# X-rayLaser/DistributedLLM

Hardware: NVIDIA H100
Metric: decode tokens/sec LLaMA-7B Q4_0 seq512 bs1 (higher is better)
Workload: dtype q4_0*q8_0->f32

## Files before the change

### distributedllm_b200/capi.py

```python
from __future__ import annotations

import ctypes as C
import os
from typing import Optional

import numpy as np

HERE = os.path.dirname(os.path.abspath(__file__))
LIB_PATH = os.path.join(HERE, "libb200slice.so")

ERRORS = {1: "EINVAL", 2: "EFILE", 3: "ENODEV", 4: "ECUDA", 5: "ECONTEXT", 6: "ENCCL"}


class B200Error(RuntimeError):
    def __init__(self, code: int, msg: str):
        super().__init__("b200 error %d (%s): %s" % (code, ERRORS.get(code, "?"), msg))
        self.code = code


class SliceInfo(C.Structure):
    _fields_ = [(n, C.c_int32) for n in ("n_embd", "n_head", "n_ff", "n_layer", "first_layer", "n_ctx", "n_past",
                                          "weight_type", "device")] + [("weight_bytes", C.c_int64),
                                                                        ("kv_bytes_per_pos", C.c_int64)]

# ... 36 lines not shown
        L.b200_slice_sync.argtypes = [vp]
        L.b200_slice_last_ms.argtypes = [vp]
        L.b200_slice_last_ms.restype = cf
        L.b200_slice_launch_count.argtypes = [vp]
        L.b200_slice_launch_count.restype = C.c_int64
        L.b200_slice_set_fast_prefill.argtypes = [vp, ci, ci]
        L.b200_slice_mark.argtypes = [vp, ci]
        L.b200_slice_mark_elapsed_ms.argtypes = [vp]
        L.b200_slice_mark_elapsed_ms.restype = cf
        L.b200_slice_profile.argtypes = [vp, ci]
        L.b200_slice_profile_read.argtypes = [vp, vp, vp, ci]
        L.b200_debug_read.argtypes = [vp, ci, C.c_size_t, C.c_size_t, vp]
        L.b200_debug_trace_enable.argtypes = [vp, ci]
        L.b200_debug_skip_attention.argtypes = [vp, ci]
        L.b200_debug_trace_read.argtypes = [vp, vp, vp, vp, ci]
        L.b200_slice_dev_in.argtypes = [vp]
        L.b200_slice_dev_in.restype = vp
        L.b200_slice_dev_out.argtypes = [vp]
        L.b200_slice_dev_out.restype = vp
        L.b200_pipeline_result.argtypes = [vp]
        L.b200_pipeline_result.restype = vp
        L.b200_device_init.argtypes = [ci]
        for name, args in (("b200_pipeline_unique_id", [vp]), ("b200_pipeline_init", [vp, ci, ci, vp]),
                           ("b200_pipeline_step", [vp, vp, ci, ci]),
                           ("b200_pipeline_mailbox_export", [vp, vp]), ("b200_pipeline_mailbox_connect", [vp, vp, ci]),
                           ("b200_pipeline_collect", [vp, ci, vp]), ("b200_pipeline_pingpong", [vp, ci, ci, vp]), ("b200_pipeline_transport", [vp]), ("b200_pipeline_set_transport", [vp, ci]), ("b200_pipeline_error", [vp]),
                           ("b200_pipeline_step_session", [vp, ci, vp, ci, ci]), ("b200_pipeline_step_batch", [vp, vp, ci, vp, ci]),
                           ("b200_pipeline_step_mixed", [vp, vp, vp, ci, vp, ci]), ("b200_pipeline_destroy", [vp]),
                           ("b200_extra_load", [C.c_char_p, ci, C.POINTER(vp)]), ("b200_extra_unload", [vp]),
                           ("b200_extra_dims", [vp, C.POINTER(ci), C.POINTER(ci)]),
# ... 153 lines not shown
        return out.view(dtype)

    def skip_attention(self, on: bool) -> None:
        check(lib().b200_debug_skip_attention(self._h, int(on)))

    def trace_enable(self, on: bool) -> None:
        check(lib().b200_debug_trace_enable(self._h, int(on)))

    def trace_read(self, max_launches: int = 512):
        buf = np.zeros((max_launches, 1024, 8), np.uint64)
        cls = np.zeros(max_launches, np.int32)
        ctas = np.zeros(max_launches, np.int32)
        n = lib().b200_debug_trace_read(self._h, _ptr(buf), _ptr(cls), _ptr(ctas), max_launches)
        return buf[:n], cls[:n], ctas[:n]

    def last_ms(self) -> float:
        return float(lib().b200_slice_last_ms(self._h))

    def launch_count(self) -> int:
        return int(lib().b200_slice_launch_count(self._h))

    def close(self) -> None:
        if self._h:
            check(lib().b200_slice_unload(self._h))
            self._h = C.c_void_p()

    def __del__(self):
        try:
            self.close()
        except Exception:
# ... 139 lines not shown
```

### distributedllm_b200/csrc/kernels.cuh

```cuda
#pragma once
#include "common.cuh"

namespace b200 {

constexpr int kWT_F16 = 1, kWT_Q4_0 = 2, kWT_Q4_1 = 3, kWT_Q5_0 = 6, kWT_Q5_1 = 7, kWT_Q8_0 = 8;
constexpr int kQ4Chunk = 576, kQ41Chunk = 640, kQ50Chunk = 704, kQ51Chunk = 768, kQ8Chunk = 1088;
constexpr int kWPC = 4;
constexpr int kConsumers = kWPC * 32;
constexpr int kQS = 4;
constexpr float kMagic = 12582912.0f;
constexpr int kMagicI = 0x4B400000;

struct WtTraits {
    int block_bytes;
    int chunk_bytes;
    bool is_signed;
    bool min_plane;
    bool high_plane;
    bool q8_1;
    float act_scale;
};
__host__ __device__ constexpr WtTraits wt_traits(int wt) {
    return wt == kWT_Q4_0 ? WtTraits{18, kQ4Chunk, true, false, false, false, 0.0625f}
         : wt == kWT_Q4_1 ? WtTraits{20, kQ41Chunk, false, true, false, true, 0.0625f}
// ... 267 lines not shown
    const int tid = threadIdx.x, warp = tid >> 5, lane = tid & 31;
    const int col0 = blockIdx.y * NC;
    const int n_stage = nbq / kQS;

    if (tid == 0) {
        B200_TRACE(a.trace, 0);
        if (RING) for (int s = 0; s < NS; s++) { mbar_init(&full[s], 1); mbar_init(&empty[s], kWPC); }
        mbar_init(actbar, 1);
        mbar_init(actbar + 1, kWPC);
        mbar_fence_init();
    }
    __syncthreads();

    if (RING && warp == kWPC) {
        if (lane == 0) {
            int slot = 0, use = 0, issued = 0;
            for (int tile = blockIdx.x; tile < a.W.n_tiles; tile += gridDim.x) {
                const uint8_t * src = a.W.data + (long long) tile * a.W.tile_bytes;
                for (int s = 0; s < n_stage; s++) {
                    if (issued == a.pre_stages) mbar_wait(actbar + 1, 0);
                    issued++;
                    if (use > 0) mbar_wait(&empty[slot], (use - 1) & 1);
                    mbar_arrive_expect_tx(&full[slot], (uint32_t) stage_bytes);
                    bulk_g2s(ring + (size_t) slot * stage_bytes, src + (size_t) s * stage_bytes, (uint32_t) stage_bytes, &full[slot]);
                    if (++slot == NS) { slot = 0; use++; }
                }
            }
            if (issued <= a.pre_stages) mbar_wait(actbar + 1, 0);
            grid_dep_launch();
            B200_TRACE(a.trace, 4);
        }
        return;
    }

    float wn[32];
    if (PRO == PRO_NORM && nb <= kConsumers) {
        #pragma unroll
        for (int j = 0; j < 8; j++) {
            const float4 u = tid < nb ? ldg_keep(a.norm_w + tid * 32 + (((NC == 1 ? tid : 0) + j) & 7) * 4) : make_float4(0.f, 0.f, 0.f, 0.f);
            wn[j*4] = u.x; wn[j*4+1] = u.y; wn[j*4+2] = u.z; wn[j*4+3] = u.w;
        }
    }
    grid_dep_wait();
    if (!RING && tid == 0) grid_dep_launch();
// ... 1323 lines not shown
```

### distributedllm_b200/csrc/kquant.cuh

```cuda
#pragma once
#include "kernels.cuh"

namespace b200 {

constexpr int kWT_Q4_K = 12;
constexpr int kQ4KChunk = 1152, kQ6KChunk = 1680;
constexpr int kKQS = 2;
static_assert(kQ4KChunk == 8 * 144 && kQ6KChunk == 8 * 210, "a chunk holds the file's bytes, nothing added");
static_assert(kQ4KChunk % 16 == 0 && kQ6KChunk % 16 == 0, "a ring stage stays one bulk copy");

__host__ __device__ constexpr bool wt_kquant(int wt) { return wt == kWT_Q4_K || wt == kWT_Q6_K; }
__host__ __device__ constexpr int kq_chunk_bytes(int wt) { return wt == kWT_Q4_K ? kQ4KChunk : kQ6KChunk; }
__host__ __device__ constexpr int kq_block_bytes(int wt) { return wt == kWT_Q4_K ? 144 : 210; }

__global__ void k_repack_kq(RepackArgs a) {
    const int cb = kq_chunk_bytes(a.wtype), words = cb / 4, bsz = kq_block_bytes(a.wtype);
    const bool q6 = a.wtype == kWT_Q6_K;
    const long long total = (long long) a.n_tiles * a.nbq * a.TR * words;
    for (long long i = blockIdx.x * (long long) blockDim.x + threadIdx.x; i < total; i += (long long) gridDim.x * blockDim.x) {
        const int wi = (int)(i % words);
        long long c = i / words;
        const int rg = (int)(c % a.TR); c /= a.TR;
        const int sb = (int)(c % a.nbq);
        const int tile = (int)(c / a.nbq);
// ... 130 lines not shown
    const int tid = threadIdx.x, warp = tid >> 5, lane = tid & 31;
    const int col0 = blockIdx.y * NC;
    const int n_stage = nbq / kKQS;

    if (tid == 0) {
        B200_TRACE(a.trace, 0);
        if (RING) for (int s = 0; s < NS; s++) { mbar_init(&full[s], 1); mbar_init(&empty[s], kWPC); }
        mbar_init(actbar, 1);
        mbar_init(actbar + 1, kWPC);
        mbar_fence_init();
    }
    __syncthreads();

    if (RING && warp == kWPC) {
        if (lane == 0) {
            int slot = 0, use = 0, issued = 0;
            for (int tile = blockIdx.x; tile < a.W.n_tiles; tile += gridDim.x) {
                const uint8_t * src = a.W.data + (long long) tile * a.W.tile_bytes;
                for (int s = 0; s < n_stage; s++) {
                    if (issued == a.pre_stages) mbar_wait(actbar + 1, 0);
                    issued++;
                    if (use > 0) mbar_wait(&empty[slot], (use - 1) & 1);
                    mbar_arrive_expect_tx(&full[slot], (uint32_t) stage_bytes);
                    bulk_g2s(ring + (size_t) slot * stage_bytes, src + (size_t) s * stage_bytes, (uint32_t) stage_bytes, &full[slot]);
                    if (++slot == NS) { slot = 0; use++; }
                }
            }
            if (issued <= a.pre_stages) mbar_wait(actbar + 1, 0);
            grid_dep_launch();
            B200_TRACE(a.trace, 4);
        }
        return;
    }

    grid_dep_wait();
    if (!RING && tid == 0) grid_dep_launch();
    if (tid == 0) B200_TRACE(a.trace, 1);

    const int ncols = min(NC, a.N - col0);
    if (tid == 0) {
        const uint32_t b1 = (uint32_t) ncols * nbq * 256, b2 = (uint32_t) ncols * nbq * 32, b3 = (uint32_t) ncols * nbd * 4;
        mbar_arrive_expect_tx(actbar, b1 + b2 + b3);
        bulk_g2s(aq_s, a.aq_in + (size_t) col0 * nbq * 64, b1, actbar);
        bulk_g2s(as_s, a.aq_in + a.in_soff + (size_t) col0 * nbq * 8, b2, actbar);
// ... 175 lines not shown
```

### distributedllm_b200/csrc/runtime.cu

```cuda
#include "kernels.cuh"
#include "kquant.cuh"
#include "fastgemm2.cuh"
#include "ggjt_file.hpp"

#include <algorithm>
#include <atomic>
#include <chrono>
#include <climits>
#include <cmath>
#include <condition_variable>
#include <dlfcn.h>
#include <cstdlib>
#include <map>
#include <memory>
#include <mutex>
#include <thread>
#include <type_traits>
#include <vector>

namespace b200 {

constexpr int kSmemLimit = 226 * 1024;

struct LayerW {
    PackedW qkv{}, wo{}, w13{}, w2{};
    PackedW qkv_more[2]{}; int qkv_row[2] = {0, 0};
    uint16_t * f_q = nullptr, * f_k = nullptr, * f_v = nullptr, * f_o = nullptr, * f_1 = nullptr, * f_2 = nullptr, * f_3 = nullptr;
    float * attn_norm = nullptr, * ffn_norm = nullptr;
};

struct GraphKey { const float * in; float * out; int host; bool operator<(const GraphKey & o) const {
    return in != o.in ? in < o.in : (out != o.out ? out < o.out : host < o.host); } };

}

using namespace b200;

struct b200_slice {
    int device = 0, n_sm = 132;
    cudaStream_t stream = nullptr;
    int E = 0, H = 0, D = 0, FF = 0, L = 0, first_layer = 0, n_ctx = 512, wtype = 0;
// ... 10 lines not shown
    uint16_t * kc = nullptr, * vc = nullptr, * q16 = nullptr;
    float * xa = nullptr, * xb = nullptr, * qkv = nullptr, * att = nullptr, * ffin = nullptr, * gate = nullptr;
    float * d_in = nullptr, * d_out = nullptr, * h_in = nullptr, * h_out = nullptr;
    float2 * cs = nullptr; uint16_t * texp = nullptr, * tsilu = nullptr;
    int * aq_att = nullptr, * aq_gate = nullptr; float * da_att = nullptr, * da_gate = nullptr;
    int nbqE = 0, nbqF = 0;
    int soffE = 0, soffF = 0;
    int * aq_x = nullptr; float * da_x = nullptr; int * nq_counter = nullptr; double * nq_partial = nullptr;
    std::map<GraphKey, cudaGraphExec_t> graphs;
    cudaEvent_t ev0 = nullptr, ev1 = nullptr; bool timed = false;
    int64_t launches = 0, weight_bytes = 0;
    bool use_ring = true, use_graph = true, use_pdl = false, use_nq = true, f16_ring = true, use_tiled_attn = true, f16_mc = true; int f16_mc_cols = 4;
    bool skip_attention = false;
    bool attn_lut_smem = true;
    bool fast_prefill = false; int fast_min_tokens = 32; uint16_t * xh = nullptr;
    int opt_ns = 0, opt_cta_per_sm = 0, opt_nc = 0, opt_pre = 3, opt_nomath = 0;
    float ema_token_ms = 0.f;
    std::mutex mu;
    bool profiling = false; int cur_class = 0;
    std::vector<cudaEvent_t> prof_ev; std::vector<int> prof_cls; size_t prof_used = 0;
    cudaEvent_t mark[2] = {nullptr, nullptr};
    unsigned long long * trace = nullptr; int trace_next = 0; std::vector<int> trace_cls, trace_ctas;
    void * nccl_comm = nullptr; int pp_rank = 0, pp_world = 1; float * d_final = nullptr;
    uint8_t * mb_block = nullptr; size_t mb_slot_floats = 0;
    uint8_t * mb_next = nullptr, * mb_prev = nullptr; bool mb_on = false;
    bool send_pending = false; PeerSendArgs send_args{}; int send_ctas = 1;
    bool fold_send = false, use_fold = true;
    int * kq_aq = nullptr; float * kq_ad = nullptr;
    std::map<GraphKey, cudaGraphExec_t> pp_graphs;
};

// ... 80 lines not shown
        m.act = kq_act_bytes(W.nbq, NC) + 34 * 8 + 64;
        return m;
    }
    m.stage = (size_t) kQS * kWPC * G * chunk_bytes(WT);
    m.act = (size_t) NC * act_bytes_per_col(W.nbq, WT) + 34 * 8 + kWPC * 8 + (size_t) NC * 128 + 64 +
            ((NC == 1 && PRO == PRO_NORM) ? (size_t) W.K * 4 : 0);
    return m;
}

template <int WT, int G, int NC, int PRO, int EPI, bool RING>
static constexpr auto gemv_kernel() {
    if constexpr (wt_kquant(WT)) return k_gemv_kq<WT, G, NC, PRO, EPI, RING>;
    else return k_gemv<WT, G, NC, PRO, EPI, RING>;
}

template <int WT, int G, int NC, int PRO, int EPI, bool RING>
static int launch_gemv_t(b200_slice * s, GemvArgs a) {
    constexpr auto kern = gemv_kernel<WT, G, NC, PRO, EPI, RING>();
    const GemvSmem sm = gemv_smem<WT, G, NC, PRO>(a.W);
    const size_t stage = sm.stage, act = sm.act;
    int NS = 0;
    if (RING) {
        const int ncolg = (a.N + NC - 1) / NC;
        int need = (a.W.n_tiles * ncolg + s->n_sm - 1) / s->n_sm;
        if (need > 5) need = 5;
        const size_t budget = (size_t) kSmemLimit / need - 1024;
        NS = s->opt_ns > 0 ? s->opt_ns : (budget > act ? (int)((budget - act) / stage) : 2);
        if (NS < 2) NS = 2;
        if (NS > 16) NS = 16;
        while (NS > 2 && NS * stage + act > (size_t) kSmemLimit) NS--;
    }
    const size_t smem = sm.bytes(NS);
    if (smem > (size_t) kSmemLimit) return fail(B200_EINVAL, "gemv needs %zu B of shared memory (K=%d, NC=%d)", smem, a.W.K, NC);
    if (int rc = smem_attr<kern>(s, kSmemLimit, true)) return rc;
    a.NS = NS; a.dbg_nomath = s->opt_nomath; a.pre_stages = s->opt_pre;
    a.trace = nullptr;
    if (s->trace && s->trace_next < 512) { a.trace = s->trace + (size_t) s->trace_next * 1024 * 8; s->trace_next++; s->trace_cls.push_back(s->cur_class); }
    int per_sm = s->opt_cta_per_sm > 0 ? s->opt_cta_per_sm : (int)(kSmemLimit / (smem + 1024));
    if (per_sm < 1) per_sm = 1;
    if (per_sm > 6) per_sm = 6;
    const int ncol = (a.N + NC - 1) / NC;
    int gx = a.W.n_tiles;
    const int cap = s->n_sm * per_sm;
    if (gx > cap) gx = cap;
    if (a.trace) s->trace_ctas.push_back(gx * ncol);
    return launch(s, kern, dim3(gx, ncol, 1), dim3(RING ? kConsumers + 32 : kConsumers, 1, 1), smem, a);
}

template <int WT, int G, int PRO, int EPI>
static int launch_gemv_nc(b200_slice * s, const GemvArgs & a) {
    if (a.N == 1) return s->use_ring ? launch_gemv_t<WT, G, 1, PRO, EPI, true>(s, a) : launch_gemv_t<WT, G, 1, PRO, EPI, false>(s, a);
    if (!s->use_ring) return launch_gemv_t<WT, G, 8, PRO, EPI, false>(s, a);
    const int want = 3 * s->n_sm, nt = a.W.n_tiles;
    const int force = s->opt_nc, cap = force > 0 ? force : 8;
    if (cap >= 8 && gemv_smem<WT, G, 8, PRO>(a.W).bytes(2) <= (size_t) kSmemLimit && (force || nt * ((a.N + 7) / 8) >= want))
        return launch_gemv_t<WT, G, 8, PRO, EPI, true>(s, a);
    if (cap >= 4 && gemv_smem<WT, G, 4, PRO>(a.W).bytes(2) <= (size_t) kSmemLimit && (force || nt * ((a.N + 3) / 4) >= want))
        return launch_gemv_t<WT, G, 4, PRO, EPI, true>(s, a);
    return launch_gemv_t<WT, G, 2, PRO, EPI, true>(s, a);
// ... 249 lines not shown
    if ((rc = attention(s, il, N, false))) return rc;
    s->cur_class = 3;
    GemvF16Args o{}; o.K = E; o.x = s->att; o.ldx = E; o.N = N; o.tsilu = s->tsilu;
    o.rows = E; o.W = Lw.f_o; o.resid = cur; o.ldr = E; o.y = s->ffin; o.ldy = E;
    if ((rc = launch_f16<PRO_PLAIN, EPI_RESID>(s, o))) return rc;
    s->cur_class = 4;
    GemvF16Args g{}; g.K = E; g.x = s->ffin; g.ldx = E; g.norm_w = Lw.ffn_norm; g.N = N; g.tsilu = s->tsilu;
    g.rows = FF; g.W = Lw.f_1; g.W2 = Lw.f_3; g.y = s->gate; g.ldy = FF;
    if ((rc = launch_f16<PRO_NORM, EPI_GATE>(s, g))) return rc;
    s->cur_class = 5;
    GemvF16Args w{}; w.K = FF; w.x = s->gate; w.ldx = FF; w.N = N; w.tsilu = s->tsilu;
    w.rows = E; w.W = Lw.f_2; w.resid = s->ffin; w.ldr = E; w.y = nxt; w.ldy = E;
    return launch_f16<PRO_PLAIN, EPI_RESID>(s, w);
}

static int layer_exact(b200_slice * s, int il, int N, const float * cur, float * nxt) {
    const int E = s->E, FF = s->FF;
    const LayerW & Lw = s->layers[il];
    const bool nq = s->use_nq && N == 1 && !s->cols && Lw.wo.n_tiles <= 256 && Lw.wo.n_tiles <= s->n_sm * 2;
    const float dsc = wt_act_scale(s->wtype);
    int rc;
    GemvArgs q{}; q.W = Lw.qkv; q.x = cur; q.ldx = E; q.norm_w = Lw.attn_norm; q.y = s->qkv; q.ldy = 3 * E;
    q.N = N; q.out_rows = 3 * E; q.tsilu = s->tsilu; q.aq_in = s->aq_x; q.da_in = s->da_x; q.in_soff = s->soffE;
    if (N > 1 && (rc = launch_norm_quant(s, cur, E, Lw.attn_norm, N))) return rc;
    if ((rc = N > 1 || (il > 0 && nq) ? launch_gemv<1, PRO_PREQ, EPI_STORE>(s, q) : launch_gemv<1, PRO_NORM, EPI_STORE>(s, q))) return rc;
    if ((rc = attention(s, il, N, true))) return rc;
    s->cur_class = 3;
    GemvArgs o{}; o.W = Lw.wo; o.x = s->att; o.ldx = E; o.resid = cur; o.ldr = E; o.y = s->ffin; o.ldy = E;
    o.N = N; o.out_rows = E; o.tsilu = s->tsilu; o.aq_in = s->aq_att; o.da_in = s->da_att; o.in_soff = s->soffE; o.out_soff = s->soffE;
    o.nq_norm_w = Lw.ffn_norm; o.nq_counter = s->nq_counter; o.nq_partial = s->nq_partial; o.aq_out = s->aq_x; o.da_out = s->da_x; o.out_nbq = s->nbqE; o.out_dscale = dsc;
    if (s->D == 128) rc = nq ? launch_gemv<1, PRO_PREQ, EPI_RESID_NQ>(s, o) : launch_gemv<1, PRO_PREQ, EPI_RESID>(s, o);
    else             rc = nq ? launch_gemv<1, PRO_PLAIN, EPI_RESID_NQ>(s, o) : launch_gemv<1, PRO_PLAIN, EPI_RESID>(s, o);
    if (rc) return rc;
    s->cur_class = 4;
    GemvArgs g{}; g.W = Lw.w13; g.x = s->ffin; g.ldx = E; g.norm_w = Lw.ffn_norm; g.y = s->gate; g.ldy = FF;
    g.N = N; g.out_rows = FF; g.tsilu = s->tsilu; g.aq_in = s->aq_x; g.da_in = s->da_x; g.in_soff = s->soffE; g.out_soff = s->soffF;
    g.aq_out = s->aq_gate; g.da_out = s->da_gate; g.out_nbq = s->nbqF; g.out_dscale = dsc;
    if (N > 1 && (rc = launch_norm_quant(s, s->ffin, E, Lw.ffn_norm, N))) return rc;
    if ((rc = N > 1 || nq ? launch_gemv<2, PRO_PREQ, EPI_GATEQ>(s, g) : launch_gemv<2, PRO_NORM, EPI_GATEQ>(s, g))) return rc;
    s->cur_class = 5;
    GemvArgs w{}; w.W = Lw.w2; w.resid = s->ffin; w.ldr = E; w.y = nxt; w.ldy = E;
    w.N = N; w.out_rows = E; w.tsilu = s->tsilu; w.aq_in = s->aq_gate; w.da_in = s->da_gate; w.in_soff = s->soffF; w.out_soff = s->soffE;
    if (il + 1 < s->L && nq) {
        w.nq_norm_w = s->layers[il + 1].attn_norm; w.nq_counter = s->nq_counter; w.nq_partial = s->nq_partial; w.aq_out = s->aq_x; w.da_out = s->da_x;
        w.out_nbq = s->nbqE; w.out_dscale = dsc;
        return launch_gemv<1, PRO_PREQ, EPI_RESID_NQ>(s, w);
    }
    if (s->fold_send && il == s->L - 1) return launch_w2_send<false>(s, w);
    return launch_gemv<1, PRO_PREQ, EPI_RESID>(s, w);
}

static int layer_fast(b200_slice * s, int il, int N, const float * cur, float * nxt) {
    const int E = s->E, FF = s->FF;
    const LayerW & Lw = s->layers[il];
    int rc;
    if ((rc = launch_prep<true>(s, cur, E, Lw.attn_norm, E, N))) return rc;
    if ((rc = launch_fast_gemm<FG_STORE>(s, Lw.qkv, nullptr, 0, s->qkv, 3 * E, N, 3 * E))) return rc;
    if ((rc = attention(s, il, N, true))) return rc;
    s->cur_class = 3;
    if ((rc = launch_prep<false>(s, s->att, E, nullptr, E, N))) return rc;
    if ((rc = launch_fast_gemm<FG_RESID>(s, Lw.wo, cur, E, s->ffin, E, N, E))) return rc;
    s->cur_class = 4;
    if ((rc = launch_prep<true>(s, s->ffin, E, Lw.ffn_norm, E, N))) return rc;
    if ((rc = launch_fast_gemm<FG_GATE>(s, Lw.w13, nullptr, 0, s->gate, FF, N, FF))) return rc;
    s->cur_class = 5;
    if ((rc = launch_prep<false>(s, s->gate, FF, nullptr, FF, N))) return rc;
    return launch_fast_gemm<FG_RESID>(s, Lw.w2, s->ffin, E, nxt, E, N, E);
}

static int layer_kquant(b200_slice * s, int il, int N, const float * cur, float * nxt) {
    const int E = s->E, FF = s->FF;
    const LayerW & Lw = s->layers[il];
    int rc;
    GemvArgs q{}; q.W = Lw.qkv; q.x = cur; q.ldx = E; q.norm_w = Lw.attn_norm; q.y = s->qkv; q.ldy = 3 * E;
    q.N = N; q.out_rows = Lw.qkv.rows; q.tsilu = s->tsilu;
    if ((rc = quant_kq(s, q, true)) || (rc = launch_gemv_kq<1, PRO_PREQ, EPI_STORE>(s, q))) return rc;
    for (int i = 0; i < 2 && Lw.qkv_more[i].data; i++) {
        q.W = Lw.qkv_more[i]; q.y = s->qkv + Lw.qkv_row[i]; q.out_rows = Lw.qkv_more[i].rows;
        if ((rc = launch_gemv_kq<1, PRO_PREQ, EPI_STORE>(s, q))) return rc;
    }
    if ((rc = attention(s, il, N, false))) return rc;
    s->cur_class = 3;
    GemvArgs o{}; o.W = Lw.wo; o.x = s->att; o.ldx = E; o.resid = cur; o.ldr = E; o.y = s->ffin; o.ldy = E;
    o.N = N; o.out_rows = E; o.tsilu = s->tsilu;
    if ((rc = quant_kq(s, o, false)) || (rc = launch_gemv_kq<1, PRO_PREQ, EPI_RESID>(s, o))) return rc;
    s->cur_class = 4;
    GemvArgs g{}; g.W = Lw.w13; g.x = s->ffin; g.ldx = E; g.norm_w = Lw.ffn_norm; g.y = s->gate; g.ldy = FF;
    g.N = N; g.out_rows = FF; g.tsilu = s->tsilu;
    if ((rc = quant_kq(s, g, true)) || (rc = launch_gemv_kq<2, PRO_PREQ, EPI_GATE>(s, g))) return rc;
    s->cur_class = 5;
    GemvArgs w{}; w.W = Lw.w2; w.x = s->gate; w.ldx = FF; w.resid = s->ffin; w.ldr = E; w.y = nxt; w.ldy = E;
    w.N = N; w.out_rows = E; w.tsilu = s->tsilu;
    if ((rc = quant_kq(s, w, false))) return rc;
    if (s->fold_send && il == s->L - 1) return launch_w2_send<true>(s, w);
    return launch_gemv_kq<1, PRO_PREQ, EPI_RESID>(s, w);
}

static int enqueue_layers(b200_slice * s, const float * in, int N, float * out) {
    const float * cur = in;
    int rc;
    for (int il = 0; il < s->L; il++) {
        const LayerW & Lw = s->layers[il];
        float * nxt = (il == s->L - 1) ? out : ((il & 1) ? s->xb : s->xa);
        const bool fast = s->fast_prefill && N > 1 && !s->cols && N >= s->fast_min_tokens &&
                          (s->wtype == kWT_Q4_0 || s->wtype == kWT_Q8_0) &&
                          (Lw.qkv.n_tiles * Lw.qkv.TR) % 16 == 0 &&
                          (Lw.wo.n_tiles * Lw.wo.TR) % 16 == 0 && (Lw.w13.n_tiles * Lw.w13.TR) % 16 == 0;
// ... 8 lines not shown
    s->cur_class = 6;
    if (s->send_pending) {
        s->send_pending = false;
        if ((rc = launch(s, k_peer_send, dim3(s->send_ctas, 1, 1), dim3(1024, 1, 1), 0, s->send_args))) return rc;
    }
    if (s->cols) return launch(s, k_advance_segs, dim3(1), dim3(32), 0, s->d_npast, s->d_segs, (int) s->segs.size());
    if (s->fold_send) return launch(s, k_advance_sent, dim3(1), dim3(32), 0, s->d_npast + s->cur, N, (MailboxHdr *) s->mb_block);
    return launch(s, k_advance, dim3(1), dim3(32), 0, s->d_npast + s->cur, N);
}

static int step_launches(const b200_slice * s) {
    int n = (s->D == 128 ? 5 : 6) * s->L + 1;
    for (const LayerW & Lw : s->layers) n += (Lw.qkv_more[0].data ? 1 : 0) + (Lw.qkv_more[1].data ? 1 : 0);
    if (wt_kquant(s->wtype)) n += 4 * s->L;
    return n;
}

static int run_decode_graph(b200_slice * s, const float * in, float * out, bool host) {
    GraphKey key{in, out, (host ? 1 : 0) | (s->skip_attention ? 2 : 0) | (s->send_pending ? 4 : 0) | (s->cur << 3)};
    auto it = s->graphs.find(key);
    const int per_step = step_launches(s);
    if (it == s->graphs.end()) {
        const int64_t before = s->launches;
        cudaGraph_t g = nullptr;
        B200_CUDA(cudaStreamBeginCapture(s->stream, cudaStreamCaptureModeThreadLocal));
        int rc = 0;
        if (host) {
            cudaMemcpyAsync(s->d_in, s->h_in, (size_t) s->E * 4, cudaMemcpyHostToDevice, s->stream);
            rc = enqueue_layers(s, s->d_in, 1, s->d_out);
            cudaMemcpyAsync(s->h_out, s->d_out, (size_t) s->E * 4, cudaMemcpyDeviceToHost, s->stream);
// ... 437 lines not shown
        if ((rc = dev_alloc(s, &s->trace, (size_t) 512 * 1024 * 8))) return rc;
        B200_CUDA(cudaMemset(s->trace, 0, (size_t) 512 * 1024 * 8 * 8));
    }
    B200_CUDA(cudaFuncSetAttribute(k_attention, cudaFuncAttributeMaxDynamicSharedMemorySize, kSmemLimit));
    B200_CUDA(cudaFuncSetAttribute(k_attn128<true>, cudaFuncAttributeMaxDynamicSharedMemorySize, 200 * 1024));
    B200_CUDA(cudaFuncSetAttribute(k_attn128<false>, cudaFuncAttributeMaxDynamicSharedMemorySize, 200 * 1024));
    if (s->D == 128) {
        cudaLaunchConfig_t cfg{};
        cfg.gridDim = dim3(4 * s->H, 1, 1); cfg.blockDim = dim3(256, 1, 1); cfg.dynamicSmemBytes = attn_need;
        int clusters = 0;
        B200_CUDA(cudaOccupancyMaxActiveClusters(&clusters, k_attn128<true>, &cfg));
        s->attn_lut_smem = clusters >= s->H;
        if (ltrace) fprintf(stderr, "[b200 load] single-token attention: %d of %d clusters resident with the exp table in shared memory: %s\n",
                            clusters, s->H, s->attn_lut_smem ? "staged" : "read through L2");
    }
    B200_CUDA(cudaEventCreate(&s->ev0));
    B200_CUDA(cudaEventCreate(&s->ev1));
    B200_CUDA(cudaDeviceSynchronize());
    lap("attributes + final sync");
    if (ltrace) fprintf(stderr, "[b200 load] total %.3f s for %.2f GB of weights\n", tnow() - t_begin, s->weight_bytes / 1e9);
    return 0;
}

static void destroy(b200_slice * s) {
    cudaSetDevice(s->device);
    if (s->stream) cudaStreamSynchronize(s->stream);
    for (auto & kv : s->graphs) cudaGraphExecDestroy(kv.second);
    for (auto & kv : s->pp_graphs) cudaGraphExecDestroy(kv.second);
    if (s->mb_next) cudaIpcCloseMemHandle(s->mb_next);
    if (s->mb_prev && s->mb_prev != s->mb_next) cudaIpcCloseMemHandle(s->mb_prev);
// ... 29 lines not shown
    if (device < 0 || device >= ndev) return fail(B200_ENODEV, "device %d out of range (%d visible)", device, ndev);
    cudaDeviceProp prop;
    B200_CUDA(cudaGetDeviceProperties(&prop, device));
    if (prop.major != 9 || prop.minor != 0) return fail(B200_ENODEV, "device %d is sm_%d%d; this library is built for sm_90a only", device, prop.major, prop.minor);
    B200_CUDA(cudaSetDevice(device));
    b200_slice * s = new b200_slice();
    s->device = device; s->n_sm = prop.multiProcessorCount;
    s->n_ctx = n_ctx > 0 ? n_ctx : 512;
    s->n_sessions = n_sessions;
    s->use_ring  = env_int("B200_RING", 1) != 0;
    s->use_graph = env_int("B200_GRAPH", 1) != 0;
    s->use_pdl   = env_int("B200_PDL", 1) != 0;
    s->fast_prefill = env_int("B200_FAST_PREFILL", 0) != 0; s->fast_min_tokens = env_int("B200_FAST_MIN_TOKENS", 32);
    s->use_nq    = env_int("B200_NQ", 0) != 0;
    s->opt_ns = env_int("B200_NS", 0); s->opt_cta_per_sm = env_int("B200_CTA_PER_SM", 0); s->opt_nc = env_int("B200_NC", 0);
    s->opt_pre = env_int("B200_PRE", 3); s->opt_nomath = env_int("B200_DBG_NOMATH", 0);
    s->use_tiled_attn = env_int("B200_TILED_ATTN", 1) != 0;
    s->f16_mc = env_int("B200_F16_MC", 1) != 0;
    s->f16_mc_cols = env_int("B200_F16_MC", 1) == 8 ? 8 : 4;
    s->f16_ring = env_int("B200_F16_RING", 1) != 0;
    cudaError_t e = cudaStreamCreateWithFlags(&s->stream, cudaStreamNonBlocking);
    if (e != cudaSuccess) { delete s; return fail(B200_ECUDA, "cudaStreamCreate failed: %s", cudaGetErrorString(e)); }
    int rc = load_locked(s, path);
    if (rc) { destroy(s); return rc; }
    *out = s;
    return 0;
}

int b200_slice_unload(b200_slice_t * s) {
    if (!s) return fail(B200_EINVAL, "null handle");
    { std::lock_guard<std::mutex> lk(s->mu); }
// ... 225 lines not shown
            else { int rc = dev_alloc(s, &s->trace, (size_t) 512 * 1024 * 8); if (rc) return rc; }
        }
        B200_CUDA(cudaMemset(s->trace, 0, (size_t) 512 * 1024 * 8 * 8));
        s->trace_next = 0; s->trace_cls.clear(); s->trace_ctas.clear();
    } else if (s->trace) { parked = s->trace; s->trace = nullptr; }
    return 0;
}

int b200_debug_trace_read(b200_slice_t * s, unsigned long long * out, int * cls, int * ctas, int max_launches) {
    if (!s || !s->trace) return 0;
    cudaSetDevice(s->device);
    cudaStreamSynchronize(s->stream);
    int n = s->trace_next < max_launches ? s->trace_next : max_launches;
    cudaMemcpy(out, s->trace, (size_t) n * 1024 * 8 * 8, cudaMemcpyDeviceToHost);
    for (int i = 0; i < n; i++) { cls[i] = s->trace_cls[i]; ctas[i] = s->trace_ctas[i]; }
    return n;
}

int b200_debug_read(b200_slice_t * s, int which, size_t offset_words, size_t count, void * out) {
    if (!s || !out) return fail(B200_EINVAL, "null argument");
    const void * src[10] = {s->qkv, s->att, s->ffin, s->gate, s->xa, s->xb, s->q16, s->kc, s->vc, s->xh};
    if (which < 0 || which > 9) return fail(B200_EINVAL, "bad buffer id %d", which);
    B200_CUDA(cudaSetDevice(s->device));
    B200_CUDA(cudaStreamSynchronize(s->stream));
    B200_CUDA(cudaMemcpy(out, (const uint32_t *) src[which] + offset_words, count * 4, cudaMemcpyDeviceToHost));
    return 0;
}

}

// ... 1227 lines not shown
```

### include/b200_slice.h

```cpp
#ifndef B200_SLICE_H
#define B200_SLICE_H

#include <stddef.h>
#include <stdint.h>

#ifdef __cplusplus
extern "C" {
#endif

typedef struct b200_slice b200_slice_t;
typedef struct b200_extra b200_extra_t;

enum {
    B200_OK       = 0,
    B200_EINVAL   = 1,
    B200_EFILE    = 2,
    B200_ENODEV   = 3,
    B200_ECUDA    = 4,
    B200_ECONTEXT = 5,
    B200_ENCCL    = 6,
};

typedef struct b200_slice_info {
    int32_t n_embd, n_head, n_ff, n_layer, first_layer, n_ctx, n_past, weight_type, device;
// ... 46 lines not shown
int b200_slice_profile(b200_slice_t * s, int enable);
int b200_slice_profile_read(b200_slice_t * s, float * ms_by_class, int * launches_by_class, int n_class);

int64_t b200_slice_launch_count(b200_slice_t * s);

float * b200_slice_dev_in(b200_slice_t * s);
float * b200_slice_dev_out(b200_slice_t * s);

int b200_debug_read(b200_slice_t * s, int which, size_t offset_words, size_t count, void * out);

int b200_debug_skip_attention(b200_slice_t * s, int on);

int b200_debug_trace_enable(b200_slice_t * s, int on);
int b200_debug_trace_read(b200_slice_t * s, unsigned long long * out, int * cls, int * ctas, int max_launches);


int b200_pipeline_unique_id(void * id128);
int b200_pipeline_init(b200_slice_t * s, int rank, int nranks, const void * id128);

int b200_pipeline_step(b200_slice_t * s, const float * d_in, int n_tokens, int ring);
int b200_pipeline_step_session(b200_slice_t * s, int session, const float * d_in, int n_tokens, int ring);
int b200_pipeline_step_batch(b200_slice_t * s, const int * sessions, int n_seq, const float * d_in, int ring);
int b200_pipeline_step_mixed(b200_slice_t * s, const int * sessions, const int * counts, int n_seq, const float * d_in, int ring);
int b200_pipeline_mailbox_export(b200_slice_t * s, void * handle64);
int b200_pipeline_mailbox_connect(b200_slice_t * s, const void * handles , int nranks);
int b200_pipeline_transport(b200_slice_t * s);
int b200_pipeline_set_transport(b200_slice_t * s, int peer);
int b200_pipeline_pingpong(b200_slice_t * s, int n_rows, int iters, float * us_per_iter);
int b200_pipeline_error(b200_slice_t * s);

// ... 41 lines not shown
```

Before: 559.3.

## Plan per-launch ring depths and release dependent grid after activation gate

Adds an optional load-time planner that picks a ring depth per decode GEMV, shrinking adjacent launches' shared-memory footprints so consecutive kernels (and attention) can co-reside on an SM under programmatic dependent launch. The producer warp now triggers grid_dep_launch right after the activation gate instead of after issuing all weight loads, letting the next kernel start earlier. The default prefetch depth before the gate changes from 3 to 5 stages (or NS when planned). The planner is off by default (env flag), but the earlier launch trigger and the new prefetch default are always on, which risks the next kernel competing for SMs and bandwidth.

```diff
diff --git a/distributedllm_b200/capi.py b/distributedllm_b200/capi.py
--- a/distributedllm_b200/capi.py
+++ b/distributedllm_b200/capi.py
@@ -74,6 +74,7 @@
         L.b200_debug_trace_enable.argtypes = [vp, ci]
         L.b200_debug_skip_attention.argtypes = [vp, ci]
         L.b200_debug_trace_read.argtypes = [vp, vp, vp, vp, ci]
+        L.b200_debug_ring_plan.argtypes = [vp, vp, ci]
         L.b200_slice_dev_in.argtypes = [vp]
         L.b200_slice_dev_in.restype = vp
         L.b200_slice_dev_out.argtypes = [vp]
@@ -257,6 +258,13 @@
         n = lib().b200_debug_trace_read(self._h, _ptr(buf), _ptr(cls), _ptr(ctas), max_launches)
         return buf[:n], cls[:n], ctas[:n]
 
+    def ring_plan(self) -> np.ndarray:
+        n = lib().b200_debug_ring_plan(self._h, None, 0)
+        check(min(n, 0))
+        out = np.zeros((n, 3), np.int32)
+        lib().b200_debug_ring_plan(self._h, _ptr(out), n)
+        return out
+
     def last_ms(self) -> float:
         return float(lib().b200_slice_last_ms(self._h))
 
diff --git a/distributedllm_b200/csrc/kernels.cuh b/distributedllm_b200/csrc/kernels.cuh
--- a/distributedllm_b200/csrc/kernels.cuh
+++ b/distributedllm_b200/csrc/kernels.cuh
@@ -305,11 +305,12 @@
 
     if (RING && warp == kWPC) {
         if (lane == 0) {
+            auto gate_then_launch = [&] { mbar_wait(actbar + 1, 0); grid_dep_launch(); };
             int slot = 0, use = 0, issued = 0;
             for (int tile = blockIdx.x; tile < a.W.n_tiles; tile += gridDim.x) {
                 const uint8_t * src = a.W.data + (long long) tile * a.W.tile_bytes;
                 for (int s = 0; s < n_stage; s++) {
-                    if (issued == a.pre_stages) mbar_wait(actbar + 1, 0);
+                    if (issued == a.pre_stages) gate_then_launch();
                     issued++;
                     if (use > 0) mbar_wait(&empty[slot], (use - 1) & 1);
                     mbar_arrive_expect_tx(&full[slot], (uint32_t) stage_bytes);
@@ -317,8 +318,7 @@
                     if (++slot == NS) { slot = 0; use++; }
                 }
             }
-            if (issued <= a.pre_stages) mbar_wait(actbar + 1, 0);
-            grid_dep_launch();
+            if (issued <= a.pre_stages) gate_then_launch();
             B200_TRACE(a.trace, 4);
         }
         return;
diff --git a/distributedllm_b200/csrc/kquant.cuh b/distributedllm_b200/csrc/kquant.cuh
--- a/distributedllm_b200/csrc/kquant.cuh
+++ b/distributedllm_b200/csrc/kquant.cuh
@@ -168,11 +168,12 @@
 
     if (RING && warp == kWPC) {
         if (lane == 0) {
+            auto gate_then_launch = [&] { mbar_wait(actbar + 1, 0); grid_dep_launch(); };
             int slot = 0, use = 0, issued = 0;
             for (int tile = blockIdx.x; tile < a.W.n_tiles; tile += gridDim.x) {
                 const uint8_t * src = a.W.data + (long long) tile * a.W.tile_bytes;
                 for (int s = 0; s < n_stage; s++) {
-                    if (issued == a.pre_stages) mbar_wait(actbar + 1, 0);
+                    if (issued == a.pre_stages) gate_then_launch();
                     issued++;
                     if (use > 0) mbar_wait(&empty[slot], (use - 1) & 1);
                     mbar_arrive_expect_tx(&full[slot], (uint32_t) stage_bytes);
@@ -180,8 +181,7 @@
                     if (++slot == NS) { slot = 0; use++; }
                 }
             }
-            if (issued <= a.pre_stages) mbar_wait(actbar + 1, 0);
-            grid_dep_launch();
+            if (issued <= a.pre_stages) gate_then_launch();
             B200_TRACE(a.trace, 4);
         }
         return;
diff --git a/distributedllm_b200/csrc/runtime.cu b/distributedllm_b200/csrc/runtime.cu
--- a/distributedllm_b200/csrc/runtime.cu
+++ b/distributedllm_b200/csrc/runtime.cu
@@ -25,6 +25,7 @@
 struct LayerW {
     PackedW qkv{}, wo{}, w13{}, w2{};
     PackedW qkv_more[2]{}; int qkv_row[2] = {0, 0};
+    int ns_qkv = 0, ns_more[2] = {0, 0}, ns_wo = 0, ns_w13 = 0, ns_w2 = 0;
     uint16_t * f_q = nullptr, * f_k = nullptr, * f_v = nullptr, * f_o = nullptr, * f_1 = nullptr, * f_2 = nullptr, * f_3 = nullptr;
     float * attn_norm = nullptr, * ffn_norm = nullptr;
 };
@@ -65,7 +66,9 @@
     bool skip_attention = false;
     bool attn_lut_smem = true;
     bool fast_prefill = false; int fast_min_tokens = 32; uint16_t * xh = nullptr;
-    int opt_ns = 0, opt_cta_per_sm = 0, opt_nc = 0, opt_pre = 3, opt_nomath = 0;
+    int opt_ns = 0, opt_cta_per_sm = 0, opt_nc = 0, opt_pre = -1, opt_nomath = 0;
+    bool use_ring_plan = false;
+    std::vector<int> ring_plan;
     float ema_token_ms = 0.f;
     std::mutex mu;
     bool profiling = false; int cur_class = 0;
@@ -176,18 +179,26 @@
     else return k_gemv<WT, G, NC, PRO, EPI, RING>;
 }
 
+static int gemv_grid_x(const b200_slice * s, int n_tiles, size_t smem) {
+    int per_sm = s->opt_cta_per_sm > 0 ? s->opt_cta_per_sm : (int)(kSmemLimit / (smem + 1024));
+    if (per_sm < 1) per_sm = 1;
+    if (per_sm > 6) per_sm = 6;
+    return std::min(n_tiles, s->n_sm * per_sm);
+}
+
 template <int WT, int G, int NC, int PRO, int EPI, bool RING>
 static int launch_gemv_t(b200_slice * s, GemvArgs a) {
     constexpr auto kern = gemv_kernel<WT, G, NC, PRO, EPI, RING>();
     const GemvSmem sm = gemv_smem<WT, G, NC, PRO>(a.W);
     const size_t stage = sm.stage, act = sm.act;
     int NS = 0;
+    const bool planned = RING && a.NS > 0;
     if (RING) {
         const int ncolg = (a.N + NC - 1) / NC;
         int need = (a.W.n_tiles * ncolg + s->n_sm - 1) / s->n_sm;
         if (need > 5) need = 5;
         const size_t budget = (size_t) kSmemLimit / need - 1024;
-        NS = s->opt_ns > 0 ? s->opt_ns : (budget > act ? (int)((budget - act) / stage) : 2);
+        NS = s->opt_ns > 0 ? s->opt_ns : planned ? a.NS : (budget > act ? (int)((budget - act) / stage) : 2);
         if (NS < 2) NS = 2;
         if (NS > 16) NS = 16;
         while (NS > 2 && NS * stage + act > (size_t) kSmemLimit) NS--;
@@ -195,16 +206,11 @@
     const size_t smem = sm.bytes(NS);
     if (smem > (size_t) kSmemLimit) return fail(B200_EINVAL, "gemv needs %zu B of shared memory (K=%d, NC=%d)", smem, a.W.K, NC);
     if (int rc = smem_attr<kern>(s, kSmemLimit, true)) return rc;
-    a.NS = NS; a.dbg_nomath = s->opt_nomath; a.pre_stages = s->opt_pre;
+    a.NS = NS; a.dbg_nomath = s->opt_nomath; a.pre_stages = s->opt_pre >= 0 ? s->opt_pre : planned ? NS : 5;
     a.trace = nullptr;
     if (s->trace && s->trace_next < 512) { a.trace = s->trace + (size_t) s->trace_next * 1024 * 8; s->trace_next++; s->trace_cls.push_back(s->cur_class); }
-    int per_sm = s->opt_cta_per_sm > 0 ? s->opt_cta_per_sm : (int)(kSmemLimit / (smem + 1024));
-    if (per_sm < 1) per_sm = 1;
-    if (per_sm > 6) per_sm = 6;
     const int ncol = (a.N + NC - 1) / NC;
-    int gx = a.W.n_tiles;
-    const int cap = s->n_sm * per_sm;
-    if (gx > cap) gx = cap;
+    const int gx = gemv_grid_x(s, a.W.n_tiles, smem);
     if (a.trace) s->trace_ctas.push_back(gx * ncol);
     return launch(s, kern, dim3(gx, ncol, 1), dim3(RING ? kConsumers + 32 : kConsumers, 1, 1), smem, a);
 }
@@ -484,14 +490,20 @@
     return launch_f16<PRO_PLAIN, EPI_RESID>(s, w);
 }
 
+static bool nq_epilogue(const b200_slice * s, const LayerW & Lw) {
+    return s->use_nq && Lw.wo.n_tiles <= 256 && Lw.wo.n_tiles <= s->n_sm * 2;
+}
+
 static int layer_exact(b200_slice * s, int il, int N, const float * cur, float * nxt) {
     const int E = s->E, FF = s->FF;
     const LayerW & Lw = s->layers[il];
-    const bool nq = s->use_nq && N == 1 && !s->cols && Lw.wo.n_tiles <= 256 && Lw.wo.n_tiles <= s->n_sm * 2;
+    const bool nq = N == 1 && !s->cols && nq_epilogue(s, Lw);
     const float dsc = wt_act_scale(s->wtype);
+    const bool step = N == 1 && !s->cols;
     int rc;
     GemvArgs q{}; q.W = Lw.qkv; q.x = cur; q.ldx = E; q.norm_w = Lw.attn_norm; q.y = s->qkv; q.ldy = 3 * E;
     q.N = N; q.out_rows = 3 * E; q.tsilu = s->tsilu; q.aq_in = s->aq_x; q.da_in = s->da_x; q.in_soff = s->soffE;
+    q.NS = step ? Lw.ns_qkv : 0;
     if (N > 1 && (rc = launch_norm_quant(s, cur, E, Lw.attn_norm, N))) return rc;
     if ((rc = N > 1 || (il > 0 && nq) ? launch_gemv<1, PRO_PREQ, EPI_STORE>(s, q) : launch_gemv<1, PRO_NORM, EPI_STORE>(s, q))) return rc;
     if ((rc = attention(s, il, N, true))) return rc;
@@ -499,6 +511,7 @@
     GemvArgs o{}; o.W = Lw.wo; o.x = s->att; o.ldx = E; o.resid = cur; o.ldr = E; o.y = s->ffin; o.ldy = E;
     o.N = N; o.out_rows = E; o.tsilu = s->tsilu; o.aq_in = s->aq_att; o.da_in = s->da_att; o.in_soff = s->soffE; o.out_soff = s->soffE;
     o.nq_norm_w = Lw.ffn_norm; o.nq_counter = s->nq_counter; o.nq_partial = s->nq_partial; o.aq_out = s->aq_x; o.da_out = s->da_x; o.out_nbq = s->nbqE; o.out_dscale = dsc;
+    o.NS = step ? Lw.ns_wo : 0;
     if (s->D == 128) rc = nq ? launch_gemv<1, PRO_PREQ, EPI_RESID_NQ>(s, o) : launch_gemv<1, PRO_PREQ, EPI_RESID>(s, o);
     else             rc = nq ? launch_gemv<1, PRO_PLAIN, EPI_RESID_NQ>(s, o) : launch_gemv<1, PRO_PLAIN, EPI_RESID>(s, o);
     if (rc) return rc;
@@ -506,11 +519,13 @@
     GemvArgs g{}; g.W = Lw.w13; g.x = s->ffin; g.ldx = E; g.norm_w = Lw.ffn_norm; g.y = s->gate; g.ldy = FF;
     g.N = N; g.out_rows = FF; g.tsilu = s->tsilu; g.aq_in = s->aq_x; g.da_in = s->da_x; g.in_soff = s->soffE; g.out_soff = s->soffF;
     g.aq_out = s->aq_gate; g.da_out = s->da_gate; g.out_nbq = s->nbqF; g.out_dscale = dsc;
+    g.NS = step ? Lw.ns_w13 : 0;
     if (N > 1 && (rc = launch_norm_quant(s, s->ffin, E, Lw.ffn_norm, N))) return rc;
     if ((rc = N > 1 || nq ? launch_gemv<2, PRO_PREQ, EPI_GATEQ>(s, g) : launch_gemv<2, PRO_NORM, EPI_GATEQ>(s, g))) return rc;
     s->cur_class = 5;
     GemvArgs w{}; w.W = Lw.w2; w.resid = s->ffin; w.ldr = E; w.y = nxt; w.ldy = E;
     w.N = N; w.out_rows = E; w.tsilu = s->tsilu; w.aq_in = s->aq_gate; w.da_in = s->da_gate; w.in_soff = s->soffF; w.out_soff = s->soffE;
+    w.NS = step ? Lw.ns_w2 : 0;
     if (il + 1 < s->L && nq) {
         w.nq_norm_w = s->layers[il + 1].attn_norm; w.nq_counter = s->nq_counter; w.nq_partial = s->nq_partial; w.aq_out = s->aq_x; w.da_out = s->da_x;
         w.out_nbq = s->nbqE; w.out_dscale = dsc;
@@ -541,26 +556,27 @@
 static int layer_kquant(b200_slice * s, int il, int N, const float * cur, float * nxt) {
     const int E = s->E, FF = s->FF;
     const LayerW & Lw = s->layers[il];
+    const bool step = N == 1 && !s->cols;
     int rc;
     GemvArgs q{}; q.W = Lw.qkv; q.x = cur; q.ldx = E; q.norm_w = Lw.attn_norm; q.y = s->qkv; q.ldy = 3 * E;
-    q.N = N; q.out_rows = Lw.qkv.rows; q.tsilu = s->tsilu;
+    q.N = N; q.out_rows = Lw.qkv.rows; q.tsilu = s->tsilu; q.NS = step ? Lw.ns_qkv : 0;
     if ((rc = quant_kq(s, q, true)) || (rc = launch_gemv_kq<1, PRO_PREQ, EPI_STORE>(s, q))) return rc;
     for (int i = 0; i < 2 && Lw.qkv_more[i].data; i++) {
-        q.W = Lw.qkv_more[i]; q.y = s->qkv + Lw.qkv_row[i]; q.out_rows = Lw.qkv_more[i].rows;
+        q.W = Lw.qkv_more[i]; q.y = s->qkv + Lw.qkv_row[i]; q.out_rows = Lw.qkv_more[i].rows; q.NS = step ? Lw.ns_more[i] : 0;
         if ((rc = launch_gemv_kq<1, PRO_PREQ, EPI_STORE>(s, q))) return rc;
     }
     if ((rc = attention(s, il, N, false))) return rc;
     s->cur_class = 3;
     GemvArgs o{}; o.W = Lw.wo; o.x = s->att; o.ldx = E; o.resid = cur; o.ldr = E; o.y = s->ffin; o.ldy = E;
-    o.N = N; o.out_rows = E; o.tsilu = s->tsilu;
+    o.N = N; o.out_rows = E; o.tsilu = s->tsilu; o.NS = step ? Lw.ns_wo : 0;
     if ((rc = quant_kq(s, o, false)) || (rc = launch_gemv_kq<1, PRO_PREQ, EPI_RESID>(s, o))) return rc;
     s->cur_class = 4;
     GemvArgs g{}; g.W = Lw.w13; g.x = s->ffin; g.ldx = E; g.norm_w = Lw.ffn_norm; g.y = s->gate; g.ldy = FF;
-    g.N = N; g.out_rows = FF; g.tsilu = s->tsilu;
+    g.N = N; g.out_rows = FF; g.tsilu = s->tsilu; g.NS = step ? Lw.ns_w13 : 0;
     if ((rc = quant_kq(s, g, true)) || (rc = launch_gemv_kq<2, PRO_PREQ, EPI_GATE>(s, g))) return rc;
     s->cur_class = 5;
     GemvArgs w{}; w.W = Lw.w2; w.x = s->gate; w.ldx = FF; w.resid = s->ffin; w.ldr = E; w.y = nxt; w.ldy = E;
-    w.N = N; w.out_rows = E; w.tsilu = s->tsilu;
+    w.N = N; w.out_rows = E; w.tsilu = s->tsilu; w.NS = step ? Lw.ns_w2 : 0;
     if ((rc = quant_kq(s, w, false))) return rc;
     if (s->fold_send && il == s->L - 1) return launch_w2_send<true>(s, w);
     return launch_gemv_kq<1, PRO_PREQ, EPI_RESID>(s, w);
@@ -599,6 +615,92 @@
     for (const LayerW & Lw : s->layers) n += (Lw.qkv_more[0].data ? 1 : 0) + (Lw.qkv_more[1].data ? 1 : 0);
     if (wt_kquant(s->wtype)) n += 4 * s->L;
     return n;
+}
+
+struct RingNode {
+    int * ns;
+    size_t stage, act; int n_tiles;
+    size_t cta_bytes; int ctas;
+};
+
+template <int G>
+static int ring_shape(const PackedW & W, bool norm, GemvSmem & m, int & n_stage) {
+    auto f = [&](auto wt) {
+        constexpr int WT = decltype(wt)::value;
+        m = norm ? gemv_smem<WT, G, 1, PRO_NORM>(W) : gemv_smem<WT, G, 1, PRO_PREQ>(W);
+        n_stage = W.nbq / (wt_kquant(WT) ? kKQS : kQS);
+        return 0;
+    };
+    return wt_kquant(W.wtype) ? with_wtype<true>(W.wtype, "k-quant matmul", f) : with_wtype<false>(W.wtype, "block-quantised matmul", f);
+}
+
+static int plan_decode_rings(b200_slice * s, bool ltrace) {
+    if (s->wtype == kWT_F16) return 0;
+    int sm_bytes = 0, reserve = 0;
+    B200_CUDA(cudaDeviceGetAttribute(&sm_bytes, cudaDevAttrMaxSharedMemoryPerMultiprocessor, s->device));
+    B200_CUDA(cudaDeviceGetAttribute(&reserve, cudaDevAttrReservedSharedMemoryPerBlock, s->device));
+    cudaFuncAttributes fa{};
+    RingNode attn{};
+    if (s->D == 128) {
+        B200_CUDA(cudaFuncGetAttributes(&fa, k_attn128<true>));
+        const AttnSmem am = attn_smem(s->n_ctx, s->D);
+        attn.cta_bytes = (s->attn_lut_smem ? am.lut : am.staged) + fa.sharedSizeBytes; attn.ctas = (4 * s->H + s->n_sm - 1) / s->n_sm;
+    } else {
+        B200_CUDA(cudaFuncGetAttributes(&fa, k_attention));
+        attn.cta_bytes = attn_smem(s->n_ctx, s->D).generic + fa.sharedSizeBytes; attn.ctas = (s->H + s->n_sm - 1) / s->n_sm;
+    }
+    std::vector<RingNode> nodes;
+    auto add = [&](const PackedW & W, int G, bool norm, int & ns) {
+        GemvSmem m; int n_stage = 0;
+        if (int rc = G == 2 ? ring_shape<2>(W, norm, m, n_stage) : ring_shape<1>(W, norm, m, n_stage)) return rc;
+        const int need = std::min(5, (W.n_tiles + s->n_sm - 1) / s->n_sm);
+        const size_t budget = (size_t) kSmemLimit / need - 1024;
+        int NS = budget > m.act ? (int)((budget - m.act) / m.stage) : 2;
+        NS = std::min({NS, 16, n_stage * ((W.n_tiles + s->n_sm * need - 1) / (s->n_sm * need))});
+        while (NS > 2 && m.bytes(NS) > (size_t) kSmemLimit) NS--;
+        ns = std::max(NS, 2);
+        nodes.push_back({&ns, m.stage, m.act, W.n_tiles, 0, 0});
+        return 0;
+    };
+    const bool kq = wt_kquant(s->wtype);
+    int rc;
+    for (int il = 0; il < s->L; il++) {
+        LayerW & Lw = s->layers[il];
+        const bool nq = !kq && nq_epilogue(s, Lw);
+        if ((rc = add(Lw.qkv, 1, !kq && !(il > 0 && nq), Lw.ns_qkv))) return rc;
+        for (int i = 0; i < 2 && Lw.qkv_more[i].data; i++) if ((rc = add(Lw.qkv_more[i], 1, false, Lw.ns_more[i]))) return rc;
+        nodes.push_back(attn);
+        if ((rc = add(Lw.wo, 1, false, Lw.ns_wo)) || (rc = add(Lw.w13, 2, !kq && !nq, Lw.ns_w13)) || (rc = add(Lw.w2, 1, false, Lw.ns_w2))) return rc;
+    }
+    auto cta_bytes = [&](const RingNode & n) { return n.ns ? n.stage * *n.ns + n.act : n.cta_bytes; };
+    auto ctas = [&](const RingNode & n) { return n.ns ? (gemv_grid_x(s, n.n_tiles, cta_bytes(n)) + s->n_sm - 1) / s->n_sm : n.ctas; };
+    auto foot = [&](const RingNode & n) { return (size_t) ctas(n) * (cta_bytes(n) + (size_t) reserve); };
+    const size_t n = nodes.size();
+    for (bool changed = true; changed;) {
+        changed = false;
+        for (size_t i = 0; i < n; i++) {
+            RingNode & p = nodes[i], & q = nodes[(i + 1) % n];
+            if (foot(p) + foot(q) <= (size_t) sm_bytes) continue;
+            RingNode * r = nullptr;
+            for (RingNode * c : {&p, &q}) if (c->ns && *c->ns > 2 && (!r || foot(*c) > foot(*r))) r = c;
+            if (r) { --*r->ns; changed = true; }
+        }
+    }
+    s->ring_plan.clear();
+    for (const RingNode & x : nodes) for (int v : {x.ns ? *x.ns : 0, ctas(x), (int) cta_bytes(x)}) s->ring_plan.push_back(v);
+    if (ltrace) {
+        const size_t per_layer = n / s->L;
+        size_t worst = 0;
+        for (size_t i = 0; i < n; i++) worst = std::max(worst, foot(nodes[i]) + foot(nodes[(i + 1) % n]));
+        fprintf(stderr, "[b200 load] single-token rings of layer 0 (NS, CTAs x KB per SM):");
+        for (size_t i = 0; i < per_layer; i++) {
+            const RingNode & x = nodes[i];
+            if (x.ns) fprintf(stderr, " NS %d %dx%.1f |", *x.ns, ctas(x), cta_bytes(x) / 1024.0);
+            else fprintf(stderr, " attention %dx%.1f |", ctas(x), cta_bytes(x) / 1024.0);
+        }
+        fprintf(stderr, " largest adjacent pair %.1f of %.1f KB per SM (%d B reserved per CTA)\n", worst / 1024.0, sm_bytes / 1024.0, reserve);
+    }
+    return 0;
 }
 
 static int run_decode_graph(b200_slice * s, const float * in, float * out, bool host) {
@@ -1066,6 +1168,7 @@
         if (ltrace) fprintf(stderr, "[b200 load] single-token attention: %d of %d clusters resident with the exp table in shared memory: %s\n",
                             clusters, s->H, s->attn_lut_smem ? "staged" : "read through L2");
     }
+    if (s->use_ring_plan && (rc = plan_decode_rings(s, ltrace))) return rc;
     B200_CUDA(cudaEventCreate(&s->ev0));
     B200_CUDA(cudaEventCreate(&s->ev1));
     B200_CUDA(cudaDeviceSynchronize());
@@ -1125,7 +1228,8 @@
     s->fast_prefill = env_int("B200_FAST_PREFILL", 0) != 0; s->fast_min_tokens = env_int("B200_FAST_MIN_TOKENS", 32);
     s->use_nq    = env_int("B200_NQ", 0) != 0;
     s->opt_ns = env_int("B200_NS", 0); s->opt_cta_per_sm = env_int("B200_CTA_PER_SM", 0); s->opt_nc = env_int("B200_NC", 0);
-    s->opt_pre = env_int("B200_PRE", 3); s->opt_nomath = env_int("B200_DBG_NOMATH", 0);
+    s->opt_pre = env_int("B200_PRE", -1); s->opt_nomath = env_int("B200_DBG_NOMATH", 0);
+    s->use_ring_plan = env_int("B200_RING_PLAN", 0) != 0;
     s->use_tiled_attn = env_int("B200_TILED_ATTN", 1) != 0;
     s->f16_mc = env_int("B200_F16_MC", 1) != 0;
     s->f16_mc_cols = env_int("B200_F16_MC", 1) == 8 ? 8 : 4;
@@ -1381,6 +1485,13 @@
     int n = s->trace_next < max_launches ? s->trace_next : max_launches;
     cudaMemcpy(out, s->trace, (size_t) n * 1024 * 8 * 8, cudaMemcpyDeviceToHost);
     for (int i = 0; i < n; i++) { cls[i] = s->trace_cls[i]; ctas[i] = s->trace_ctas[i]; }
+    return n;
+}
+
+int b200_debug_ring_plan(b200_slice_t * s, int * out, int max_launches) {
+    if (!s) return fail(B200_EINVAL, "b200_debug_ring_plan: null slice");
+    const int n = (int)(s->ring_plan.size() / 3);
+    if (out) std::copy(s->ring_plan.begin(), s->ring_plan.begin() + 3 * std::min(n, std::max(max_launches, 0)), out);
     return n;
 }
 
diff --git a/include/b200_slice.h b/include/b200_slice.h
--- a/include/b200_slice.h
+++ b/include/b200_slice.h
@@ -84,6 +84,8 @@
 int b200_debug_trace_enable(b200_slice_t * s, int on);
 int b200_debug_trace_read(b200_slice_t * s, unsigned long long * out, int * cls, int * ctas, int max_launches);
 
+int b200_debug_ring_plan(b200_slice_t * s, int * out, int max_launches);
+
 
 int b200_pipeline_unique_id(void * id128);
 int b200_pipeline_init(b200_slice_t * s, int rank, int nranks, const void * id128);
```

Result: faster. 570.8, median of 6 (+2.1%).
